# takah29/3d-reconstruction-from-multi-view-exp

Measured on AMD Instinct MI355X. Metric: BA iterations/sec + residual-Jacobian GObs/s, 1M pts x 100 cams fp64, higher is better.
Workload: dtype f64

## Files before the change

3d-reconstruction-from-multi-view-exp_amd/csrc/host_check.cpp:

```cpp
#include <algorithm>
#include <cmath>
#include <cstdio>
#include <cstring>
#include <iterator>
#include <limits>
#include <string>
#include <vector>

#include "mvba_host.h"
#include "mvba_engine_host.h"
#include "mvba_ransac_host.h"
#include "mvba_tracks_host.h"
#include "mvba_match_host.h"

namespace mvba {
thread_local std::string g_err;
}
using namespace mvba;

static int failures = 0;
#define CHECK(x) do { if (!(x)) { std::printf("host_check: line %d: %s\n", __LINE__, #x); ++failures; } } while (0)

int main() {
  {
// ... 796 lines not shown
    auto cost_threads = [](int m) { return std::min(512, table_block_threads(sizeof(double) * (size_t)CAM_LDS * m)); };
    CHECK(k5_bytes(182) == 40768 && k5_bytes(183) == 40992 && k5_bytes(365) == 81760 && k5_bytes(366) == 81984);
    CHECK(table_block_threads(k5_bytes(182)) == 256 && table_block_threads(k5_bytes(183)) == 512);
    CHECK(table_block_threads(k5_bytes(365)) == 512 && table_block_threads(k5_bytes(366)) == 1024);
    CHECK(table_block_threads(40 * 1024) == 256 && table_block_threads(80 * 1024) == 512 && table_block_threads(0) == 256);
    CHECK(cost_threads(284) == 256 && cost_threads(285) == 512 && cost_threads(646) == 512);
    CHECK(k5_lanes(40.0) == 2 && k5_lanes(std::nextafter(40.0, 41.0)) == 4 && k5_lanes(100.0) == 4 && k5_lanes(std::nextafter(100.0, 101.0)) == 8 && k5_lanes(1.0) == 2);
    CHECK(cov_lanes(12.0) == 8 && cov_lanes(std::nextafter(12.0, 13.0)) == 16 && cov_lanes(24.0) == 16 && cov_lanes(std::nextafter(24.0, 25.0)) == 32);
    CHECK(cov_lanes(48.0) == 32 && cov_lanes(std::nextafter(48.0, 49.0)) == 64 && cov_lanes(0.0) == 8);
    auto in = [](auto &dom, int v) { return std::find(std::begin(dom), std::end(dom), v) != std::end(dom); };
    for (double d : {1.0, 40.0, 41.0, 100.0, 101.0, 1e6}) CHECK(in(K5_LANES, k5_lanes(d)));
    for (size_t by : {(size_t)0, (size_t)40961, (size_t)81921, (size_t)160 * 1024}) CHECK(in(TABLE_BLOCK_THREADS, table_block_threads(by)));
    for (double pr : {0.0, 13.0, 25.0, 49.0, 1e6}) CHECK(in(COV_LANES, cov_lanes(pr)));
    CHECK(std::size(K5_LANES) == 3 && std::size(TABLE_BLOCK_THREADS) == 3 && std::size(COV_LANES) == 4);
  }
  if (failures) return 1;
  std::printf("host_check ok\n");
  return 0;
}
```

3d-reconstruction-from-multi-view-exp_amd/csrc/mvba_create.h:

```cpp

__global__ __launch_bounds__(256) void k_xy_from_planes(const double2 *__restrict__ planes, long long N, int m, double2 *__restrict__ xy) {
  const long long a = (long long)blockIdx.x * 256 + threadIdx.x;
  const int k = blockIdx.y;
  if (a < N) xy[a * m + k] = planes[(long long)k * N + a];
}

#define CR(x) do { int rc_ = (x); if (rc_) return rc_; } while (0)

struct CreateTimer {
  bool on;
  std::chrono::steady_clock::time_point t_last = std::chrono::steady_clock::now();
  void lap(const char *what) {
    if (!on) return;
    const auto now = std::chrono::steady_clock::now();
    fprintf(stderr, "mvba_create: %-28s %8.1f ms\n", what, std::chrono::duration<double, std::milli>(now - t_last).count());
    t_last = now;
  }
};

int validate_problem(const mvba_problem *p, std::vector<int> &obs_pt) {
  if (p->n_points < 0 || p->n_images < 2 || p->n_obs < 0 || !p->pt_ptr || (p->n_obs && (!p->cam_idx || !p->xy)))
    return fail(MVBA_ERR_BADARG, "bad problem sizes or null arrays (need n_images >= 2)");
  if (p->gauge_axis != 0 && p->gauge_axis != 1) return fail(MVBA_ERR_BADARG, "gauge_axis must be 0 or 1");
  if (p->xy_layout != 0 && p->xy_layout != 1) return fail(MVBA_ERR_BADARG, "xy_layout must be 0 (observation order) or 1 (image planes)");
// ... 121 lines not shown
    L.n_diag_lists += L.S[pair_id(m, k, k)];
    for (int l = k + 1; l < m; ++l) L.n_off_lists += L.S[pair_id(m, k, l)];
  }
  L.vp_off.assign(L.VP + 1, 0);
  for (long long q = 0; q < P; ++q)
    for (int sI = 0; sI < L.S[q]; ++sI) L.vp_off[L.vp_ptr[q] + sI + 1] = (L.cnt[q] - sI + L.S[q] - 1) / L.S[q];
  for (int v = 0; v < L.VP; ++v) L.vp_off[v + 1] += L.vp_off[v];
  return MVBA_OK;
}

struct PointRanges {
  int nR = 1;
  std::vector<long long> lo;
};

PointRanges make_ranges(const IndexInput &in, const PairLists &L, bool slots, int xcd_waves, int W) {
  PointRanges R;
  const long long N = in.N;
  if (slots) {
    const long long j = std::max<long long>(1, std::min<long long>(xcd_waves / std::max(1LL, L.slot_waves(W)), L.target / (8 * 64)));
    R.nR = (int)(8 * std::min<long long>(j, 8));
    R.lo.assign(R.nR + 1, 0);
    std::vector<long long> pre(N + 1, 0);
    for (long long a = 0; a < N; ++a) {
      const long long d = in.p->pt_ptr[a + 1] - in.p->pt_ptr[a];
      pre[a + 1] = pre[a] + d * (d + 1) / 2;
    }
    for (int r = 0; r <= R.nR; ++r)
      R.lo[r] = std::lower_bound(pre.begin(), pre.end(), (long long)((__int128)pre[N] * r / R.nR)) - pre.begin();
    R.lo[0] = 0; R.lo[R.nR] = N;
  } else {
    const long long nR_big = (L.target + L.unit_items / 2) / L.unit_items, nR_fill = std::min<long long>((4096 + L.VP - 1) / L.VP, L.target / 128);
    R.nR = (int)std::max<long long>(1, std::min<long long>(64, std::max(nR_big, nR_fill)));
    R.lo.assign(R.nR + 1, 0);
    for (int r = 0; r <= R.nR; ++r) R.lo[r] = (long long)((__int128)N * r / R.nR);
  }
  return R;
}

constexpr long long LANES_SKEW = 12288;
constexpr long long LANES_MIN_WAVES = 78;

struct SchurPlan {
  int mode = SCHUR_SLOTS;
  int W = PSTEP;
  std::vector<int> dense_obs;
  PairLists L;
  PointRanges R;
};

template <typename CountPairs>
int decide_schur_form(const IndexInput &in, const CreateKnobs &knobs, int loss, int device, CountPairs count_pairs, SchurPlan &plan,
                      CreateTimer &timer) {
  const mvba_problem *p = in.p;
  const long long N = in.N, nobs = in.nobs;
  const int m = in.m;
  {
    bool few = m >= 1 && 9 * m <= 16 * DENSE_MAX_TILES && N > 0, full = few && nobs == N * (long long)m;
    for (long long a = 0; a < N && full; ++a) {
      if (p->pt_ptr[a + 1] - p->pt_ptr[a] != m) { full = false; break; }
      const int *ci = p->cam_idx + p->pt_ptr[a];
      for (int k = 0; k < m; ++k)
        if (ci[k] != k) { full = false; break; }
    }
    const bool forced = knobs.schur_dense;
    bool masked = few && !full && (forced || (!knobs.schur_set && (double)nobs >= 0.6 * (double)N * m)) && (long long)N * m < (1LL << 31);
    if (masked) {
      plan.dense_obs.assign((size_t)N * m, -1);
// ... 9 lines not shown
    if ((full && (!knobs.schur_set || forced)) || masked) {
      plan.mode = SCHUR_DENSE;
      return MVBA_OK;
    }
  }
  plan.L.cnt.assign(in.P, 0);
  CR(count_pairs(plan.L.cnt));
  timer.lap("pair counts");
  CR(size_pair_lists(in, plan.L));
  const PairLists &L = plan.L;
  int n_cu_dev = 256;
  hipDeviceGetAttribute(&n_cu_dev, hipDeviceAttributeMultiprocessorCount, device);
  auto xcd_waves = [&](int W) { return std::max(1, n_cu_dev / 8) * (W == LANES_W ? 160 * 1024 / LANES_LDS : 160 * 1024 / SLOT_LDS); };
  const bool slots_forced = knobs.schur_slots || knobs.schur_lanes;
  const bool may_slots = !knobs.schur_pairs && loss == LOSS_SQUARED && (N + 1) * 128LL < (1LL << 32) && !knobs.force_big && (L.T >= 4000000 || slots_forced);
  auto slot_plan = [&](int W, PointRanges &R) {
    if (!may_slots || L.slot_waves(W) > xcd_waves(W)) return false;
    R = make_ranges(in, L, true, xcd_waves(W), W);
    if (W == PSTEP && !slots_forced && R.nR * L.slot_waves(W) < 512) return false;
    long long widest = 0;
    for (int r = 0; r < R.nR; ++r) widest = std::max<long long>(widest, p->pt_ptr[R.lo[r + 1]] - p->pt_ptr[R.lo[r]]);
    return (widest + 1) * 128LL < (1LL << 32);
  };
  PointRanges R21, R64;
  const bool fits21 = slot_plan(PSTEP, R21);
  const bool lanes = knobs.schur_lanes ? slot_plan(LANES_W, R64)
                                       : (fits21 && !knobs.schur_slots && L.slot_waves(LANES_W) >= LANES_MIN_WAVES && slot_plan(LANES_W, R64));
  if (lanes) {
    plan.mode = SCHUR_SLOTS; plan.W = LANES_W; plan.R = std::move(R64);
  } else if (fits21) {
    plan.mode = SCHUR_SLOTS; plan.W = PSTEP; plan.R = std::move(R21);
  } else {
    plan.mode = SCHUR_PAIRS;
    plan.R = make_ranges(in, L, false, 0, PSTEP);
  }
  return MVBA_OK;
}
// ... 559 lines not shown
  MVBA_HIP(hipGetDevice(&h->device));
  MVBA_HIP(hipStreamCreateWithFlags(&h->stream, hipStreamNonBlocking));
  CR(h->mem.alloc(&h->d_pt_ptr, N + 1));
  CR(h->mem.alloc(&h->d_cam, nobs));
  MVBA_HIP(hipMemcpy(h->d_pt_ptr, p->pt_ptr, sizeof(long long) * (N + 1), hipMemcpyHostToDevice));
  if (nobs) MVBA_HIP(hipMemcpy(h->d_cam, p->cam_idx, sizeof(int) * nobs, hipMemcpyHostToDevice));
  timer.lap("device, topology upload");
  h->k1_threads = k1_block_threads(m, h->gcam);

  const bool dev_build = N > 0 && nobs > 0 && !knobs.index_host;
  const IndexInput in{p, N, nobs, (long long)m * (m + 1) / 2, m,
                      (int)std::max(1u, std::min({std::thread::hardware_concurrency(), 16u, (unsigned)m})), h->stream, h->d_pt_ptr, h->d_cam};
  DeviceIndexBuild dv;
  SchurPlan plan;
  SchurIndex ix;
  CR(decide_schur_form(in, knobs, h->loss, h->device, [&](std::vector<long long> &cnt) {
    return dev_build ? count_pairs_device(in, knobs, dv, cnt) : count_pairs_host(in, cnt);
  }, plan, timer));
  h->schur_mode = plan.mode;
  h->use_pairs = plan.mode != SCHUR_DENSE;
  h->rec_compact = plan.mode == SCHUR_SLOTS && plan.W == LANES_W && h->loss == LOSS_SQUARED && !h->gcam && !knobs.rec_full;
  if (h->use_pairs) CR(dev_build ? build_index_device(in, plan, dv, h->mem, ix, timer) : build_index_host(in, plan, h->mem, ix, timer));
  timer.lap("queues / wave descriptors");

  CR(alloc_engine_buffers(h, tiles));
  timer.lap("allocations");
  CR(upload_engine(h, p, obs_pt, tiles, plan, ix));
  timer.lap("uploads");
  CR(set_kernel_attributes(h, knobs));
  timer.lap("attributes");
  return MVBA_OK;
}

int create_engine(const mvba_problem *p, int loss, double loss_b, mvba_handle **out) {
  if (!p || !out) return fail(MVBA_ERR_BADARG, "null argument");
  const CreateKnobs knobs = read_create_knobs();
// ... 27 lines not shown
```

3d-reconstruction-from-multi-view-exp_amd/csrc/mvba_debug.h:

```cpp
#include <functional>

extern "C" {

namespace {
constexpr int SNAP_SLAB = 8;
size_t snap_stride(const mvba_handle *h) { return (3 * (size_t)h->N + (size_t)CAM_IN * h->m + 1) & ~(size_t)1; }
double *snap_entry(const mvba_handle *h, long long i) { return h->snap_slabs[(size_t)(i / SNAP_SLAB)] + snap_stride(h) * (size_t)(i % SNAP_SLAB); }
}

int mvba_snapshot(mvba_handle *h) {
  if (!h) return fail(MVBA_ERR_BADARG, "null handle");
  if (!h->have_params) return fail(MVBA_ERR_STATE, "no parameters set");
  MVBA_HIP(hipSetDevice(h->device));
  if ((size_t)(h->n_snap / SNAP_SLAB) >= h->snap_slabs.size()) {
    double *p = nullptr;
    int rc = h->mem.alloc(&p, snap_stride(h) * SNAP_SLAB);
    if (rc) return rc;
    h->snap_slabs.push_back(p);
  }
  double *dst = snap_entry(h, h->n_snap);
  MVBA_HIP(hipMemcpyAsync(dst, h->d_X[h->cur], sizeof(double) * 3 * h->N, hipMemcpyDeviceToDevice, h->stream));
  MVBA_HIP(hipMemcpyAsync(dst + 3 * h->N, h->d_cam15[h->cur], sizeof(double) * CAM_IN * h->m, hipMemcpyDeviceToDevice, h->stream));
  h->n_snap++;
  return MVBA_OK;
// ... 36 lines not shown
int mvba_get_stats(mvba_handle *h, mvba_stats *out) {
  if (!h || !out) return fail(MVBA_ERR_BADARG, "null argument");
  MVBA_HIP(hipSetDevice(h->device));
  int rc = sync_and_drain(h);
  if (rc) return rc;
  *out = h->stats;
  return MVBA_OK;
}

int mvba_get_info(mvba_handle *h, int64_t *out8) {
  if (!h || !out8) return fail(MVBA_ERR_BADARG, "null argument");
  out8[0] = h->n_items;
  out8[1] = h->n_items_offdiag;
  out8[2] = h->n_units;
  out8[3] = h->schur_mode | (h->schur_mode == SCHUR_SLOTS ? h->slot_w << 8 : 0) | (h->rec_compact ? 1 << 16 : 0) |
            (h->schur_mode == SCHUR_DENSE ? (int64_t)h->dense_blocks << 32 : 0);
  out8[4] = h->rccl_version;
  out8[5] = NCCL_VERSION_CODE;
  out8[6] = h->nranks;
  out8[7] = h->schur_mode == SCHUR_SLOTS ? h->n_slot_items : 0;
  return MVBA_OK;
}

int mvba_reset_stats(mvba_handle *h) {
  if (!h) return fail(MVBA_ERR_BADARG, "null handle");
  MVBA_HIP(hipSetDevice(h->device));
  int rc = sync_and_drain(h);
  if (rc) return rc;
  h->stats = mvba_stats{};
  return MVBA_OK;
// ... 54 lines not shown
}

int debug_fill_A(mvba_handle *h, double *out) {
  std::vector<double> pk(h->n_A());
  MVBA_HIP(hipMemcpy(pk.data(), h->d_Ab, sizeof(double) * pk.size(), hipMemcpyDeviceToHost));
  expand_packed_A(pk.data(), h->m, out);
  return MVBA_OK;
}

int debug_fill_index(mvba_handle *h, int which, long long cnt, double *out) {
  if (h->schur_mode == SCHUR_SLOTS && which != MVBA_BUF_INDEX_SEG) {
    const int W = h->slot_w, row = slot_idx_ints(W);
    const long long n_steps = cnt / W;
    std::vector<int> tmp((size_t)n_steps * row);
    if (cnt) MVBA_HIP(hipMemcpy(tmp.data(), h->d_it_x, sizeof(int) * tmp.size(), hipMemcpyDeviceToHost));
    const int off = which == MVBA_BUF_INDEX_K ? 0 : (which == MVBA_BUF_INDEX_L ? W : 2 * W);
    for (long long st = 0; st < n_steps; ++st)
      for (int sl = 0; sl < W; ++sl) out[st * W + sl] = (double)tmp[(size_t)st * row + off + sl];
    return MVBA_OK;
  }
  const int *src = which == MVBA_BUF_INDEX_K ? h->d_it_k : (which == MVBA_BUF_INDEX_L ? h->d_it_l : (which == MVBA_BUF_INDEX_A ? h->d_it_a : h->d_seg_end));
  std::vector<int> tmp((size_t)cnt);
  if (cnt) MVBA_HIP(hipMemcpy(tmp.data(), src, sizeof(int) * tmp.size(), hipMemcpyDeviceToHost));
  for (long long i = 0; i < cnt; ++i) out[i] = (double)tmp[i];
  return MVBA_OK;
}

DebugBuf debug_buffer(mvba_handle *h, int which) {
  const long long N = h->N, nobs = h->nobs, n9 = (long long)h->n9();
  switch (which) {
// ... 36 lines not shown
```

3d-reconstruction-from-multi-view-exp_amd/csrc/mvba_engine.h:

```cpp
enum { SCHUR_PAIRS = 1, SCHUR_SLOTS = 2, SCHUR_DENSE = 3 };
struct mvba_handle {
  int device = 0;
  hipStream_t stream = nullptr;
  DevBufs mem;
  long long N = 0, nobs = 0;
  int m = 0, gauge_axis = 0, D = 0, ld = 0;
  double f0 = 1.0;
  long long *d_pt_ptr = nullptr;
  int *d_cam = nullptr, *d_obs_pt = nullptr;
  double2 *d_xy = nullptr;
  int *d_tiles = nullptr;
  int *d_tile_slot = nullptr;
  int4 *d_splits = nullptr;
  double *d_PLsplit = nullptr;
  int n_splits = 0;
  int n_tiles = 0;
  bool any_split = false;
  int k1_threads = 512;
  bool gcam = false;
  double *d_cam18 = nullptr, *d_dxi10 = nullptr;
  bool use_pairs = true;
  int schur_mode = 2;
  bool index_on_device = false;
  bool force_big = false;
  long long n_items = 0, n_items_offdiag = 0, n_slot_items = 0;
  int n_units = 0, q_max = 0;
  int *d_it_k = nullptr, *d_it_l = nullptr, *d_it_a = nullptr, *d_unit_ptr = nullptr, *d_q_ptr = nullptr, *d_q_units = nullptr;
  int4 *d_units = nullptr;
  double *d_partial = nullptr;
  int n_waves = 0, slot_nR = 8, slot_nseg = 0;
  int slot_w = PSTEP;
  long long *d_range_o0 = nullptr;
  int *d_seg_end = nullptr, *d_prog = nullptr;
  int4 *d_wdesc = nullptr;
  int *d_it_x = nullptr;
  int *d_wunits = nullptr;
  double *d_dense_part = nullptr;
  int *d_dense_obs = nullptr;
  int dense_blocks = 0, dense_tiles = 0;
  double *d_X[2] = {nullptr, nullptr}, *d_cam15[2] = {nullptr, nullptr};
  int cur = 0;
  bool have_params = false, linearized = false, have_trial = false;
  double *d_sim = nullptr;
  double2 *d_rec = nullptr;
  bool rec_compact = false;
  double2 *d_res = nullptr, *d_rec_full = nullptr;
// ... 261 lines not shown
  const size_t lds = cam_lds_bytes(h->m, h->gcam, false);
  cam_tables(h, cam15, nullptr);
  launch_loss(h, cost_kernel(h->gcam, h->loss), dim3(h->cost_grid), dim3(std::min(512, table_block_threads(lds))), lds, h->nobs, h->m, cam15, X,
              h->d_obs_pt, h->d_cam, h->d_xy, h->f0, h->d_partials, h->d_cam18);
  double *mail = cost_mail(h);
  const unsigned long long seq = h->cost_seq;
  hipLaunchKernelGGL(k_sum_partials, dim3(1), dim3(1024), 0, h->stream, h->d_partials, h->cost_grid, h->d_cost, h->d_flag, mail, seq);
  MVBA_HIP(hipGetLastError());
  return MVBA_OK;
}

struct CreateKnobs {
  bool schur_set = false;
  bool schur_slots = false, schur_lanes = false, schur_pairs = false, schur_dense = false;
  bool index_host = false, index_global = false;
  bool force_big = false;
  bool rec_full = false;
  bool chol_launches = false;
  int trail64_min = 200;
  unsigned barrier_polls = 1u << 22;
  bool check_solve = false;
  double check_solve_tol = 1e-8;
  bool timing = false;
};

CreateKnobs read_create_knobs() {
  CreateKnobs k;
  auto is = [](const char *ev, const char *v) { return ev && !strcmp(ev, v); };
  const char *schur = getenv("MVBA_SCHUR");
  k.schur_set = schur != nullptr;
  k.schur_slots = is(schur, "slots");
  k.schur_lanes = is(schur, "lanes");
  k.schur_pairs = is(schur, "pairs");
  k.schur_dense = is(schur, "dense");
  const char *index = getenv("MVBA_INDEX");
  k.index_host = is(index, "host");
  k.index_global = is(index, "global");
  k.force_big = getenv("MVBA_FORCE_BIG") != nullptr;
  k.rec_full = is(getenv("MVBA_REC"), "full");
  k.chol_launches = is(getenv("MVBA_CHOL"), "launches");
  if (const char *ev = getenv("MVBA_TRAIL64_MIN")) k.trail64_min = std::max(0, atoi(ev));
  if (const char *ev = getenv("MVBA_CHOL_BARRIER_POLLS")) k.barrier_polls = (unsigned)std::max(0LL, atoll(ev));
  if (const char *ev = getenv("MVBA_CHECK_SOLVE")) {
    const double v = atof(ev);
    k.check_solve = v != 0.0;
    if (v > 0.0 && v < 1.0) k.check_solve_tol = v;
  }
  k.timing = getenv("MVBA_CREATE_TIMING") != nullptr;
  return k;
}

}
// ... 1 lines not shown
```

3d-reconstruction-from-multi-view-exp_amd/csrc/mvba_engine_host.h:

```cpp
#pragma once
#include <algorithm>
#include <cmath>
#include <cstddef>
#include <string>
#include <vector>

#include "mvba_common.h"

namespace mvba {

inline bool is_gauge_slot(long long g, int axis) { return (g >= 3 && g <= 8) || g == 12 + axis; }

struct ParameterMap {
  bool is_default = false;
  std::vector<int> ptr, mem;
  std::vector<int2> pairs;
  int U = 0, nblk = 1;
};

inline int build_parameter_map(const int32_t *col, int m, int axis, int n_free, int D, ParameterMap &out) {
  const int n9 = 9 * m;
  if (n_free < 0 || n_free > D)
    return fail(MVBA_ERR_BADARG, "mvba_set_parameter_map: n_free = " + std::to_string(n_free) + " must be in 0 .. 9 n_images - 7 = " + std::to_string(D));
  std::vector<int> cnt(n_free + 1, 0), first(n_free, -1);
// ... 109 lines not shown
    double *c = cam + (size_t)k * CAM_IN;
    c[0] = f[k]; c[1] = u[2 * k]; c[2] = u[2 * k + 1];
    for (int i = 0; i < 3; ++i) c[3 + i] = t[3 * k + i];
    for (int i = 0; i < 9; ++i) c[6 + i] = R[9 * k + i];
  }
}
inline void unpack_cam15(const double *cam , int m, double *f, double *u, double *t, double *R) {
  for (int k = 0; k < m; ++k) {
    const double *c = cam + (size_t)k * CAM_IN;
    f[k] = c[0]; u[2 * k] = c[1]; u[2 * k + 1] = c[2];
    for (int i = 0; i < 3; ++i) t[3 * k + i] = c[3 + i];
    for (int i = 0; i < 9; ++i) R[9 * k + i] = c[6 + i];
  }
}

constexpr int K5_LANES[] = {2, 4, 8};
inline int k5_lanes(double mean_degree) { return mean_degree <= 40.0 ? 2 : (mean_degree <= 100.0 ? 4 : 8); }
constexpr int TABLE_BLOCK_THREADS[] = {256, 512, 1024};
inline int table_block_threads(size_t lds_bytes) { return lds_bytes > 80 * 1024 ? 1024 : (lds_bytes > 40 * 1024 ? 512 : 256); }
constexpr int COV_LANES[] = {8, 16, 32, 64};
inline int cov_lanes(double mean_pairs) { return mean_pairs > 48.0 ? 64 : (mean_pairs > 24.0 ? 32 : (mean_pairs > 12.0 ? 16 : 8)); }

}
```

3d-reconstruction-from-multi-view-exp_amd/csrc/mvba_index.h:

```cpp

constexpr int IDX_WAVES = 4;

__device__ __forceinline__ int idx_pair_id(int k, int l, int m) { return k * m - k * (k - 1) / 2 + (l - k); }

template <bool GLOBAL>
__global__ __launch_bounds__(64 * IDX_WAVES) void k_idx_count(long long N, int m, int P, const long long *__restrict__ pt_ptr,
                                                              const int *__restrict__ cam_idx, int chunk,
                                                              int *__restrict__ hist, const int *__restrict__ order) {
  extern __shared__ int s_hist_all[];
  const int lane = threadIdx.x & 63, wv = threadIdx.x >> 6;
  const long long w = (long long)blockIdx.x * IDX_WAVES + wv;
  int *s_hist = GLOBAL ? hist + (size_t)w * P : s_hist_all + (size_t)wv * P;
  if (!GLOBAL) {
    for (int q = lane; q < P; q += 64) s_hist[q] = 0;
    wave_sync();
  }
  const long long a0 = w * chunk, a1 = min(N, a0 + chunk);
  for (long long ai = a0; ai < a1; ++ai) {
    const long long a = order ? order[ai] : ai;
    const long long o0 = pt_ptr[a];
    const int d = (int)(pt_ptr[a + 1] - o0);
    for (int i = 0; i < d; ++i) {
      const int k = cam_idx[o0 + i];
      for (int j = i + lane; j < d; j += 64) {
// ... 121 lines not shown
  }
  if (FILL) {
    if (lane == 0)
      while (sg < nSeg) seg_end[b * nSeg + sg++] = steps;
  } else if (lane == 0) {
    w_steps[b] = steps;
  }
}

__global__ void k_idx_interleave(long long n_steps, int W, int row, const int *__restrict__ st_k, const int *__restrict__ st_l,
                                 const int *__restrict__ st_a, int *__restrict__ out) {
  const long long t = (long long)blockIdx.x * blockDim.x + threadIdx.x;
  if (t >= n_steps * row) return;
  const long long st = t / row;
  const int e = (int)(t - st * row), which = e / W, sl = e - which * W;
  const int *src = which == 0 ? st_k : (which == 1 ? st_l : st_a);
  out[t] = which < 3 ? src[st * W + sl] : 0;
}
```

3d-reconstruction-from-multi-view-exp_amd/csrc/mvba_lanes.h:

```cpp
#pragma once

constexpr int LANES_W = 64;
constexpr int LANES_IDX = 3 * LANES_W;
constexpr int LANES_BUF = SchurStage<LANES_W, false, true>::SIZE;
constexpr int LANES_LDS = 3 * LANES_BUF + 2 * LANES_IDX * 4;
static_assert(LANES_BUF == 17408 && LANES_LDS == 53760, "the launch's LDS bytes");
static_assert(SchurStage<LANES_W, true, true>::SIZE <= LANES_BUF, "a diagonal step fits the buffer");
static_assert(3 * ((LANES_LDS + 511) / 512 * 512) <= 160 * 1024, "three waves per CU");
constexpr int LANES_BUF_C = SchurStage<LANES_W, false, true, true>::SIZE;
constexpr int LANES_LDS_C = 3 * LANES_BUF_C + 2 * LANES_IDX * 4;
static_assert(LANES_BUF_C == 13312 && LANES_LDS_C == 41472, "the compact launch's LDS bytes");
static_assert(SchurStage<LANES_W, true, true, true>::SIZE == 12288, "a compact diagonal step fits the buffer");
static_assert(3 * ((LANES_LDS_C + 511) / 512 * 512) <= 160 * 1024 && 4 * ((LANES_LDS_C + 511) / 512 * 512) > 160 * 1024, "three waves per CU");

struct LanesCompact {
  const double2 *res = nullptr;
  const int4 *units = nullptr;
  const double *cam15 = nullptr;
};
template <int SH>
__device__ __forceinline__ void lds_gather16_rows(int row, unsigned slot16, const void *base, unsigned lds) {
  unsigned o;
  asm volatile("s_mov_b32 m0, %4\n\tv_lshl_add_u32 %0, %1, %5, %2\n\tglobal_load_lds_dwordx4 %0, %3" : "=&v"(o) : "v"(row), "v"(slot16), "s"(base), "s"(lds), "i"(SH) : "memory");
}
template <int G>
__device__ __forceinline__ void lanes_wait() {
  static_assert(G == 12 || G == 13 || G == 17, "the loops of k_schur_lanes and k_schur_lanes_compact");
  if (G == 12) asm volatile("s_waitcnt vmcnt(12)" ::: "memory");
// ... 9 lines not shown
  using S = SchurStage<LANES_W, DIAG, true, COMPACT>;
  constexpr int NPS = S::NPS, BUFSZ = S::SIZE, NBUF = 3;
  constexpr int RSL = COMPACT ? 4 : 7;
  constexpr int G = DIAG ? RSL + 1 + NPS : RSL + RSL + NPS;
  double acc[9][9];
#pragma unroll
  for (int i = 0; i < 9; ++i)
#pragma unroll
    for (int j = 0; j < 9; ++j) acc[i][j] = 0.0;
  double dg[9], rb[9];
#pragma unroll
  for (int j = 0; j < 9; ++j) dg[j] = rb[j] = 0.0;

  const unsigned lds0 = (unsigned)(unsigned long long)(__attribute__((address_space(3))) char *)wbuf;
  const unsigned ldsx0 = lds0 + NBUF * BUFSZ;
  const int *xring = reinterpret_cast<const int *>(wbuf + NBUF * BUFSZ);
  const int *xbase = it_x + beg * LANES_IDX;
  const int last_st = nst - 1;
  auto rec_row = [&](int j) { return (64 * j + lane) / RSL; };
  auto rec_s16 = [&](int j) { return COMPACT ? (unsigned)((lane & 3) ^ ((lane >> 4) & 3)) << 4 : (unsigned)((64 * j + lane) % 7) << 4; };
  auto pb_row = [&](int j) { return (64 * j + lane) / NPS; };
  auto pb_s16 = [&](int j) { return (unsigned)(COMPACT ? ((64 * j + lane) % NPS + 6) & 7 : (64 * j + lane) % NPS) << 4; };
  const unsigned lane16 = (unsigned)min(lane, 47) << 4;
  auto index_row = [&](int st, unsigned ring_off) {
    const int *src = xbase + (size_t)min(st, last_st) * LANES_IDX;
    const unsigned dst = ldsx0 + ring_off;
    if (lane < 48) lds_index_row(lane16, src, dst);
  };
  constexpr unsigned RING_B = LANES_IDX * 4;
  auto issue_step = [&](unsigned ring_off, unsigned ring_next, unsigned buf_off, int st_idx) {
    index_row(st_idx, ring_next);
    const int *x = reinterpret_cast<const int *>(reinterpret_cast<const char *>(xring) + ring_off);
    const unsigned buf = lds0 + buf_off;
    int kx[RSL], ax[NPS], lx[RSL];
#pragma unroll
    for (int j = 0; j < RSL; ++j) kx[j] = x[rec_row(j)];
#pragma unroll
    for (int j = 0; j < NPS; ++j) ax[j] = x[2 * LANES_W + pb_row(j)];
#pragma unroll
    for (int j = 0; j < RSL; ++j) lx[j] = DIAG ? (j == 0 ? x[lane] : 0) : x[LANES_W + rec_row(j)];
#pragma unroll
    for (int j = 0; j < RSL; ++j) asm volatile("" : "+v"(kx[j]), "+v"(lx[j]));
#pragma unroll
    for (int j = 0; j < NPS; ++j) asm volatile("" : "+v"(ax[j]));
    if constexpr (COMPACT) {
#pragma unroll
      for (int j = 0; j < RSL; ++j) {
        lds_gather16_rows<6>(kx[j], rec_s16(j), rec, buf + 1024 * j);
        if (!DIAG) lds_gather16_rows<6>(lx[j], rec_s16(j), rec, buf + S::L + 1024 * j);
      }
      if (DIAG) lds_gather16_rows<4>(lx[0], 0u, cx.res, buf + S::L);
    } else if (!DIAG) {
#pragma unroll
      for (int j = 0; j < 7; ++j) {
        lds_gather16(kx[j], rec_s16(j), rec, buf + 1024 * j);
        lds_gather16(lx[j], rec_s16(j), rec, buf + S::L + 1024 * j);
      }
    } else {
#pragma unroll
// ... 118 lines not shown
```

3d-reconstruction-from-multi-view-exp_amd/csrc/mvba_schur.h:

```cpp


constexpr int PSTEP = 21;
constexpr int PROW = 7 * 16;
constexpr int UNIT_STRIDE = 104;
constexpr int SLOT_IDX = 64;
constexpr int SLOT_IDX_RING = 3;

template <int W, bool DIAG, bool PACKED, bool COMPACT = false>
struct SchurStage {
  static_assert(!COMPACT || PACKED, "the compact rows are the slot forms'");
  static constexpr int ROW = COMPACT ? 4 * 16 : PROW;
  static constexpr int NPS = (DIAG ? 5 : 3) + (COMPACT ? 2 : 0);
  static constexpr int L = W * ROW;
  static constexpr int P = L + ((PACKED && DIAG) ? W * 16 : W * ROW);
  static constexpr int SIZE = P + W * 16 * (PACKED ? NPS : 5);
  static constexpr int SQW = DIAG ? L + W * 16 : P + W * 16 * NPS;
  static constexpr int SQW_END = SQW + (DIAG ? 1 : 2) * W * 8;
};
constexpr int PWAVE_LDS = SchurStage<PSTEP, false, false>::SIZE;
constexpr int SLOT_BUF = SchurStage<PSTEP, false, true>::SIZE;
constexpr int PAIRS_LDS = 2 * PWAVE_LDS;
constexpr int SLOT_LDS = 3 * SLOT_BUF + SLOT_IDX_RING * SLOT_IDX * 4;
static_assert(PWAVE_LDS == 6384 && SLOT_BUF == 5712 && SLOT_LDS == 17904, "the launches' LDS bytes");
static_assert(SchurStage<PSTEP, true, false>::SIZE == PWAVE_LDS && SchurStage<PSTEP, true, true>::SIZE <= SLOT_BUF, "a diagonal step fits the buffer");
// ... 428 lines not shown
      double *__restrict__ partial, int nR, const int *__restrict__ seg_end, int *__restrict__ prog,                      \
      int nseg, int lag, const long long *__restrict__ range_o0
__global__ __launch_bounds__(64, 3) void k_schur_slots(MVBA_SLOTS_ARGS) {
  schur_slots_wave(wdesc, wunits, it_k, it_l, it_a, rec, PB, c, f0, partial, nR, seg_end, prog, nseg, lag, range_o0);
}

#include "mvba_lanes.h"
constexpr int slot_idx_ints(int W) { return W == LANES_W ? LANES_IDX : SLOT_IDX; }

__global__ __launch_bounds__(64, 1) void k_schur_lanes(const int4 *__restrict__ wdesc, const int *__restrict__ wunits,
                                                       const int *__restrict__ it_x, const double2 *__restrict__ rec,
                                                       const double *__restrict__ PB, double c, double f0,
                                                       double *__restrict__ partial, int nR,
                                                       const long long *__restrict__ range_o0) {
  extern __shared__ char smem_pairs[];
  const int bid = blockIdx.x;
  const int MVBA_CONST_AS *dp = as_const(reinterpret_cast<const int *>(wdesc)) + 4 * (size_t)bid;
  const int d_x = dp[0], d_y = dp[1], nsteps = dp[2], flags = dp[3];
  if (nsteps <= 0) return;
  const long long beg = ((long long)d_y << 32) | (unsigned)d_x;
  const int *su = wunits + (size_t)bid * LANES_W;
  const double2 *rec_r = rec + (size_t)as_const(range_o0)[bid % nR] * REC;
  if (flags & 1) schur_lanes_run<true>(smem_pairs, (int)threadIdx.x, beg, nsteps, it_x, rec_r, PB, c, 1.0 / f0, partial, su);
  else schur_lanes_run<false>(smem_pairs, (int)threadIdx.x, beg, nsteps, it_x, rec_r, PB, c, 1.0 / f0, partial, su);
}
__global__ __launch_bounds__(64, 1) void k_schur_lanes_compact(const int4 *__restrict__ wdesc, const int *__restrict__ wunits,
                                                               const int *__restrict__ it_x, const double2 *__restrict__ rec,
                                                               const double *__restrict__ PB, double c, double f0,
                                                               double *__restrict__ partial, int nR,
                                                               const long long *__restrict__ range_o0, const double2 *__restrict__ res,
                                                               const int4 *__restrict__ units, const double *__restrict__ cam15) {
  extern __shared__ char smem_pairs[];
  const int bid = blockIdx.x;
  const int MVBA_CONST_AS *dp = as_const(reinterpret_cast<const int *>(wdesc)) + 4 * (size_t)bid;
  const int d_x = dp[0], d_y = dp[1], nsteps = dp[2], flags = dp[3];
  if (nsteps <= 0) return;
  const long long beg = ((long long)d_y << 32) | (unsigned)d_x;
  const int *su = wunits + (size_t)bid * LANES_W;
  const long long o0 = as_const(range_o0)[bid % nR];
  const LanesCompact cx{res + o0, units, cam15};
  if (flags & 1) schur_lanes_run<true, true>(smem_pairs, (int)threadIdx.x, beg, nsteps, it_x, rec + (size_t)o0 * REC_C, PB, c, 1.0 / f0, partial, su, cx);
  else schur_lanes_run<false, true>(smem_pairs, (int)threadIdx.x, beg, nsteps, it_x, rec + (size_t)o0 * REC_C, PB, c, 1.0 / f0, partial, su, cx);
}

__global__ __launch_bounds__(128) void k_schur_reduce(int m, const int *__restrict__ unit_ptr,
                                                      const double *__restrict__ partial, double *__restrict__ Afull,
                                                      double *__restrict__ bfull) {
  const long long p = blockIdx.x;
// ... 32 lines not shown
```

3d-reconstruction-from-multi-view-exp_amd/lib/_mvba.py:

```python
from __future__ import annotations

import ctypes as C
import os
import threading

import numpy as np

_HERE = os.path.dirname(os.path.abspath(__file__))
LIB_PATH = os.environ.get("MVBA_LIBRARY", os.path.join(os.path.dirname(_HERE), "libmvba.so"))

MVBA_OK, MVBA_ERR_BADARG, MVBA_ERR_SINGULAR, MVBA_ERR_HIP, MVBA_ERR_RCCL, MVBA_ERR_STATE = range(6)

KERNEL_IDS = ("resid_jac", "point_blocks", "point_inv", "schur", "allreduce", "solve", "backsub_cost", "cost")
BUF = {"residual": 0, "JX": 1, "JC": 2, "E": 3, "dP": 4, "A_full": 5, "b_full": 6, "dxi": 7, "dX": 8,
       "trial_X": 9, "trial_cam": 10, "index_k": 11, "index_l": 12, "index_a": 13, "index_seg": 14, "weight": 15}
LOSSES = {"squared": 0, "huber": 1, "cauchy": 2}


def check_loss(loss, loss_scale):
    if not isinstance(loss, str) or loss not in LOSSES:
        raise ValueError(f"loss must be one of {sorted(LOSSES)}, got {loss!r}")
    if loss == "squared":
        return 0, 0.0
    if loss_scale is None:
# ... 367 lines not shown
        raise_for(self.lib.mvba_get_stats(self._h, C.byref(s)), self.lib)
        out = {k: {"ms": s.ms[i], "launches": s.launches[i]} for i, k in enumerate(KERNEL_IDS)}
        out["counts"] = {"linearize": s.n_linearize, "try_step": s.n_try_step, "commit": s.n_commit,
                         "lu_fallback": s.n_lu_fallback, "barrier_fallback": s.n_barrier_fallback}
        return out

    def _info(self):
        out = (C.c_int64 * 8)()
        raise_for(self.lib.mvba_get_info(self._h, out), self.lib)
        return list(out)

    def schur_info(self):
        i = self._info()
        return {"items": i[0], "offdiag_items": i[1], "units": i[2], "kernel": ("strip", "pairs", "slots", "dense")[i[3] & 0xff],
                "slot_rows": i[7], "step_width": (i[3] >> 8) & 0xff,
                "record": "compact" if (i[3] >> 16) & 1 else "full",
                "workgroups": i[3] >> 32}

    def rccl_version(self):
        i = self._info()
        return {"loaded": i[4], "compiled_against": i[5], "ranks": i[6]}

    def comm_init(self, id128: bytes, rank: int, n_ranks: int):
        buf = C.create_string_buffer(bytes(id128), 128)
        raise_for(self.lib.mvba_comm_init(self._h, buf, int(rank), int(n_ranks)), self.lib)

    def comm_init_host(self, rank: int, n_ranks: int, allreduce):
        HOSTFN = C.CFUNCTYPE(C.c_int, C.c_void_p, _dp, C.c_int64)

        def _cb(_user, buf, n):
# ... 544 lines not shown
```

Before: 453.8.

## Pack lane Schur indices into two words and size ranges by occupancy

The (k, l, a) index triple for each 64-wide lane step is packed into two 32-bit words instead of three. This shrinks the per-block LDS index ring so the compact lanes kernel fits four waves per CU instead of three. The number of point ranges is now derived from the measured occupancy (blocks per CU times CU count) rather than a fixed multiple of eight. Blocks are remapped to range waves so that each range stays on its home XCD. The cost is extra bit unpacking per step, a range limit on N and degree for the packed format, and a lower LANES_MIN_WAVES threshold that may change which Schur kernel is selected.

After: 486.9 (median of 6 runs). +7.3%, better.

```diff
diff --git a/3d-reconstruction-from-multi-view-exp_amd/csrc/host_check.cpp b/3d-reconstruction-from-multi-view-exp_amd/csrc/host_check.cpp
--- a/3d-reconstruction-from-multi-view-exp_amd/csrc/host_check.cpp
+++ b/3d-reconstruction-from-multi-view-exp_amd/csrc/host_check.cpp
@@ -834,6 +834,72 @@
     for (double pr : {0.0, 13.0, 25.0, 49.0, 1e6}) CHECK(in(COV_LANES, cov_lanes(pr)));
     CHECK(std::size(K5_LANES) == 3 && std::size(TABLE_BLOCK_THREADS) == 3 && std::size(COV_LANES) == 4);
   }
+  {
+    const int ROW = (int)LANE_IDX_MAX_ROW, OFF = (int)LANE_IDX_MAX_OFF;
+    CHECK(LANE_IDX_ROW_BITS == 25 && LANE_IDX_OFF_BITS == 14 && ROW == (1 << 25) - 1 && OFF == 16383);
+    auto round_trip = [](int k, int l, int a) {
+      int k2 = -1, l2 = -1, a2 = -1;
+      const LaneIdx p = lane_idx_pack(k, l, a);
+      lane_idx_unpack(p, k2, l2, a2);
+      return k2 == k && l2 == l && a2 == a && lane_idx_k(p.w0) == k && lane_idx_l(p.w0, p.w1) == l && lane_idx_a(p.w1) == a;
+    };
+    const int ks[] = {0, 1, 127, 128, (1 << 24) + 5, ROW - OFF, ROW - 1, ROW}, as[] = {0, 1, 77, 1 << 24, ROW - 1, ROW};
+    const int ds[] = {0, 1, 63, 64, 79, 127, 128, 129, 255, 256, 8191, 8192, OFF - 1, OFF};
+    for (int k : ks)
+      for (int d : ds)
+        for (int a : as)
+          if ((long long)k + d <= ROW) CHECK(round_trip(k, k + d, a));
+    CHECK(round_trip(ROW - OFF, ROW, ROW));
+    {
+      const int N = 1234567;
+      const LaneIdx pad = lane_idx_pack(0, 0, N), dg = lane_idx_pack(4711, 4711, 42);
+      CHECK(pad.w0 == 0u && pad.w1 == (unsigned)N && round_trip(0, 0, N) && round_trip(0, 0, ROW));
+      CHECK(dg.w0 == 4711u && dg.w1 == 42u && lane_idx_l(dg.w0, dg.w1) == lane_idx_k(dg.w0));
+    }
+    CHECK(lane_idx_pack(0, 127, 0).w0 == 127u << 25 && lane_idx_pack(0, 127, 0).w1 == 0u);
+    CHECK(lane_idx_pack(0, 128, 0).w0 == 0u && lane_idx_pack(0, 128, 0).w1 == 1u << 25);
+    CHECK(lane_idx_pack(ROW - OFF, ROW, ROW).w1 == 0xffffffffu);
+    static_assert(lane_idx_l(lane_idx_pack(5, 300, 9).w0, lane_idx_pack(5, 300, 9).w1) == 300, "constexpr on the host and in the kernels");
+    const long long NMAX = (1LL << 32) / 128 - 2;
+    CHECK((NMAX + 1) * 128 < (1LL << 32) && (NMAX + 2) * 128 >= (1LL << 32));
+    CHECK(lane_idx_fits(NMAX, NMAX, 16384) && !lane_idx_fits(NMAX, NMAX, 16385) && lane_idx_fits(0, 0, 0) && lane_idx_fits(10, 20, 1));
+    CHECK(!lane_idx_fits(ROW + 1, 10, 2) && !lane_idx_fits(10, ROW + 2, 2) && lane_idx_fits(ROW, ROW + 1, 2));
+  }
+  {
+    const long long T = 10000;
+    CHECK(lane_ranges(1024, 95, T, 0) == 10 && lane_ranges(768, 95, T, 0) == 8);
+    CHECK(lane_ranges(1024, 78, T, 0) == 13 && lane_ranges(1024, 63, T, 0) == 16 && lane_ranges(1024, 96, T, 0) == 10);
+    CHECK(lane_ranges(1024, 1024, T, 0) == 1 && lane_ranges(1024, 1025, T, 0) == 1 && lane_ranges(1024, 513, T, 0) == 1 && lane_ranges(1024, 512, T, 0) == 2);
+    CHECK(lane_ranges(1000, 96, T, 0) == 10 && lane_ranges(959, 96, T, 0) == 9);
+    CHECK(lane_ranges(1024, 1, T, 0) == 64 && lane_ranges(1024, 9, 1LL << 40, 0) == 64 && lane_ranges(1024, 9, 1024, 0) == 16 && lane_ranges(1024, 9, 1023, 0) == 8);
+    CHECK(lane_ranges(1024, 9, 0, 0) == 8 && lane_ranges(1024, 200, 0, 0) == 5 && lane_ranges(0, 9, T, 0) == 1 && lane_ranges(1024, 0, T, 0) == 64);
+    CHECK(lane_ranges(1024, 95, T, 1) == 1 && lane_ranges(1024, 95, T, 3) == 3 && lane_ranges(1024, 95, T, 11) == 11 && lane_ranges(768, 95, 0, 64) == 64);
+    CHECK(lane_ranges(1024, 95, T, 65) == LANE_MAX_RANGES && lane_ranges(1024, 95, T, 1 << 30) == LANE_MAX_RANGES);
+  }
+  {
+    for (int nR : {1, 3, 7, 8, 9, 10, 11, 15, 16, 17, 23, 64})
+      for (int rw : {1, 2, 9, 95, 96}) {
+        const int T = nR * rw, q = nR / 8;
+        std::vector<int> seen(T, 0), surplus(8, 0);
+        bool home_ok = true, same = true, order = true;
+        std::vector<int> last_w(nR, -1);
+        for (int B = 0; B < T; ++B) {
+          const int b = lane_wave_of_block(B, nR, rw);
+          if (b < 0 || b >= T) { home_ok = false; continue; }
+          ++seen[b];
+          const int r = b % nR, w = b / nR;
+          if (r < 8 * q) home_ok = home_ok && B % 8 == r % 8;
+          else ++surplus[B % 8];
+          same = same && b == B;
+          order = order && w > last_w[r];
+          last_w[r] = w;
+        }
+        CHECK(std::all_of(seen.begin(), seen.end(), [](int c) { return c == 1; }));
+        CHECK(home_ok && order);
+        CHECK(*std::max_element(surplus.begin(), surplus.end()) - *std::min_element(surplus.begin(), surplus.end()) <= 1);
+        CHECK(same || (nR % 8 != 0 && nR > 8));
+      }
+  }
   if (failures) return 1;
   std::printf("host_check ok\n");
   return 0;
diff --git a/3d-reconstruction-from-multi-view-exp_amd/csrc/mvba_create.h b/3d-reconstruction-from-multi-view-exp_amd/csrc/mvba_create.h
--- a/3d-reconstruction-from-multi-view-exp_amd/csrc/mvba_create.h
+++ b/3d-reconstruction-from-multi-view-exp_amd/csrc/mvba_create.h
@@ -159,12 +159,12 @@
   std::vector<long long> lo;
 };
 
-PointRanges make_ranges(const IndexInput &in, const PairLists &L, bool slots, int xcd_waves, int W) {
+PointRanges make_ranges(const IndexInput &in, const PairLists &L, bool slots, int xcd_waves, int W, int lane_nR = 0) {
   PointRanges R;
   const long long N = in.N;
   if (slots) {
     const long long j = std::max<long long>(1, std::min<long long>(xcd_waves / std::max(1LL, L.slot_waves(W)), L.target / (8 * 64)));
-    R.nR = (int)(8 * std::min<long long>(j, 8));
+    R.nR = W == LANES_W ? std::max(1, lane_nR) : (int)(8 * std::min<long long>(j, 8));
     R.lo.assign(R.nR + 1, 0);
     std::vector<long long> pre(N + 1, 0);
     for (long long a = 0; a < N; ++a) {
@@ -184,7 +184,7 @@
 }
 
 constexpr long long LANES_SKEW = 12288;
-constexpr long long LANES_MIN_WAVES = 78;
+constexpr long long LANES_MIN_WAVES = 38;
 
 struct SchurPlan {
   int mode = SCHUR_SLOTS;
@@ -192,11 +192,12 @@
   std::vector<int> dense_obs;
   PairLists L;
   PointRanges R;
+  int lane_places = 0;
 };
 
 template <typename CountPairs>
-int decide_schur_form(const IndexInput &in, const CreateKnobs &knobs, int loss, int device, CountPairs count_pairs, SchurPlan &plan,
-                      CreateTimer &timer) {
+int decide_schur_form(const IndexInput &in, const CreateKnobs &knobs, int loss, bool compact_rec, int device, CountPairs count_pairs,
+                      SchurPlan &plan, CreateTimer &timer) {
   const mvba_problem *p = in.p;
   const long long N = in.N, nobs = in.nobs;
   const int m = in.m;
@@ -236,13 +237,23 @@
   auto xcd_waves = [&](int W) { return std::max(1, n_cu_dev / 8) * (W == LANES_W ? 160 * 1024 / LANES_LDS : 160 * 1024 / SLOT_LDS); };
   const bool slots_forced = knobs.schur_slots || knobs.schur_lanes;
   const bool may_slots = !knobs.schur_pairs && loss == LOSS_SQUARED && (N + 1) * 128LL < (1LL << 32) && !knobs.force_big && (L.T >= 4000000 || slots_forced);
+  int lane_places = 0;
+  if (may_slots)
+    MVBA_HIP(hipOccupancyMaxActiveBlocksPerMultiprocessor(&lane_places, compact_rec ? (const void *)k_schur_lanes_compact : (const void *)k_schur_lanes, 64,
+                                                          compact_rec ? LANES_LDS_C : LANES_LDS));
+  lane_places = std::max(1, lane_places);
+  plan.lane_places = lane_places;
+  long long max_degree = 0;
+  for (long long a = 0; a < N; ++a) max_degree = std::max<long long>(max_degree, p->pt_ptr[a + 1] - p->pt_ptr[a]);
   auto slot_plan = [&](int W, PointRanges &R) {
     if (!may_slots || L.slot_waves(W) > xcd_waves(W)) return false;
-    R = make_ranges(in, L, true, xcd_waves(W), W);
+    R = make_ranges(in, L, true, xcd_waves(W), W,
+                    lane_ranges((long long)n_cu_dev * lane_places, L.slot_waves(LANES_W), L.target, knobs.slot_ranges));
     if (W == PSTEP && !slots_forced && R.nR * L.slot_waves(W) < 512) return false;
     long long widest = 0;
     for (int r = 0; r < R.nR; ++r) widest = std::max<long long>(widest, p->pt_ptr[R.lo[r + 1]] - p->pt_ptr[R.lo[r]]);
-    return (widest + 1) * 128LL < (1LL << 32);
+    if ((widest + 1) * 128LL >= (1LL << 32)) return false;
+    return W != LANES_W || lane_idx_fits(N, widest, max_degree);
   };
   PointRanges R21, R64;
   const bool fits21 = slot_plan(PSTEP, R21);
@@ -832,12 +843,14 @@
   DeviceIndexBuild dv;
   SchurPlan plan;
   SchurIndex ix;
-  CR(decide_schur_form(in, knobs, h->loss, h->device, [&](std::vector<long long> &cnt) {
+  const bool compact_rec = h->loss == LOSS_SQUARED && !h->gcam && !knobs.rec_full;
+  CR(decide_schur_form(in, knobs, h->loss, compact_rec, h->device, [&](std::vector<long long> &cnt) {
     return dev_build ? count_pairs_device(in, knobs, dv, cnt) : count_pairs_host(in, cnt);
   }, plan, timer));
   h->schur_mode = plan.mode;
   h->use_pairs = plan.mode != SCHUR_DENSE;
-  h->rec_compact = plan.mode == SCHUR_SLOTS && plan.W == LANES_W && h->loss == LOSS_SQUARED && !h->gcam && !knobs.rec_full;
+  h->rec_compact = plan.mode == SCHUR_SLOTS && plan.W == LANES_W && compact_rec;
+  h->lane_places = plan.mode == SCHUR_SLOTS && plan.W == LANES_W ? plan.lane_places : 0;
   if (h->use_pairs) CR(dev_build ? build_index_device(in, plan, dv, h->mem, ix, timer) : build_index_host(in, plan, h->mem, ix, timer));
   timer.lap("queues / wave descriptors");
 
diff --git a/3d-reconstruction-from-multi-view-exp_amd/csrc/mvba_debug.h b/3d-reconstruction-from-multi-view-exp_amd/csrc/mvba_debug.h
--- a/3d-reconstruction-from-multi-view-exp_amd/csrc/mvba_debug.h
+++ b/3d-reconstruction-from-multi-view-exp_amd/csrc/mvba_debug.h
@@ -74,6 +74,7 @@
   out8[1] = h->n_items_offdiag;
   out8[2] = h->n_units;
   out8[3] = h->schur_mode | (h->schur_mode == SCHUR_SLOTS ? h->slot_w << 8 : 0) | (h->rec_compact ? 1 << 16 : 0) |
+            (h->schur_mode == SCHUR_SLOTS ? (int64_t)(h->slot_nR & 0xff) << 20 | (int64_t)(h->lane_places & 0xf) << 28 : 0) |
             (h->schur_mode == SCHUR_DENSE ? (int64_t)h->dense_blocks << 32 : 0);
   out8[4] = h->rccl_version;
   out8[5] = NCCL_VERSION_CODE;
@@ -158,6 +159,15 @@
     const long long n_steps = cnt / W;
     std::vector<int> tmp((size_t)n_steps * row);
     if (cnt) MVBA_HIP(hipMemcpy(tmp.data(), h->d_it_x, sizeof(int) * tmp.size(), hipMemcpyDeviceToHost));
+    if (W == LANES_W) {
+      for (long long st = 0; st < n_steps; ++st)
+        for (int sl = 0; sl < W; ++sl) {
+          int k, l, a;
+          lane_idx_unpack({(unsigned)tmp[(size_t)st * row + sl], (unsigned)tmp[(size_t)st * row + W + sl]}, k, l, a);
+          out[st * W + sl] = (double)(which == MVBA_BUF_INDEX_K ? k : (which == MVBA_BUF_INDEX_L ? l : a));
+        }
+      return MVBA_OK;
+    }
     const int off = which == MVBA_BUF_INDEX_K ? 0 : (which == MVBA_BUF_INDEX_L ? W : 2 * W);
     for (long long st = 0; st < n_steps; ++st)
       for (int sl = 0; sl < W; ++sl) out[st * W + sl] = (double)tmp[(size_t)st * row + off + sl];
diff --git a/3d-reconstruction-from-multi-view-exp_amd/csrc/mvba_engine.h b/3d-reconstruction-from-multi-view-exp_amd/csrc/mvba_engine.h
--- a/3d-reconstruction-from-multi-view-exp_amd/csrc/mvba_engine.h
+++ b/3d-reconstruction-from-multi-view-exp_amd/csrc/mvba_engine.h
@@ -30,6 +30,7 @@
   double *d_partial = nullptr;
   int n_waves = 0, slot_nR = 8, slot_nseg = 0;
   int slot_w = PSTEP;
+  int lane_places = 0;
   long long *d_range_o0 = nullptr;
   int *d_seg_end = nullptr, *d_prog = nullptr;
   int4 *d_wdesc = nullptr;
@@ -321,6 +322,7 @@
   bool schur_set = false;
   bool schur_slots = false, schur_lanes = false, schur_pairs = false, schur_dense = false;
   bool index_host = false, index_global = false;
+  int slot_ranges = 0;
   bool force_big = false;
   bool rec_full = false;
   bool chol_launches = false;
@@ -343,6 +345,7 @@
   const char *index = getenv("MVBA_INDEX");
   k.index_host = is(index, "host");
   k.index_global = is(index, "global");
+  if (const char *ev = getenv("MVBA_SLOT_RANGES")) k.slot_ranges = std::max(0, atoi(ev));
   k.force_big = getenv("MVBA_FORCE_BIG") != nullptr;
   k.rec_full = is(getenv("MVBA_REC"), "full");
   k.chol_launches = is(getenv("MVBA_CHOL"), "launches");
diff --git a/3d-reconstruction-from-multi-view-exp_amd/csrc/mvba_engine_host.h b/3d-reconstruction-from-multi-view-exp_amd/csrc/mvba_engine_host.h
--- a/3d-reconstruction-from-multi-view-exp_amd/csrc/mvba_engine_host.h
+++ b/3d-reconstruction-from-multi-view-exp_amd/csrc/mvba_engine_host.h
@@ -147,6 +147,41 @@
   }
 }
 
+constexpr int LANE_IDX_ROW_BITS = 25, LANE_IDX_OFF_BITS = 2 * (32 - LANE_IDX_ROW_BITS);
+constexpr unsigned LANE_IDX_ROW_MASK = (1u << LANE_IDX_ROW_BITS) - 1, LANE_IDX_OFF_LOW = (1u << (32 - LANE_IDX_ROW_BITS)) - 1;
+constexpr long long LANE_IDX_MAX_ROW = LANE_IDX_ROW_MASK, LANE_IDX_MAX_OFF = (1LL << LANE_IDX_OFF_BITS) - 1;
+struct LaneIdx { unsigned w0, w1; };
+__host__ __device__ constexpr LaneIdx lane_idx_pack(int k, int l, int a) {
+  const unsigned d = (unsigned)(l - k);
+  return {(unsigned)k | (d & LANE_IDX_OFF_LOW) << LANE_IDX_ROW_BITS, (unsigned)a | (d >> (32 - LANE_IDX_ROW_BITS)) << LANE_IDX_ROW_BITS};
+}
+__host__ __device__ constexpr int lane_idx_k(unsigned w0) { return (int)(w0 & LANE_IDX_ROW_MASK); }
+__host__ __device__ constexpr int lane_idx_a(unsigned w1) { return (int)(w1 & LANE_IDX_ROW_MASK); }
+__host__ __device__ constexpr int lane_idx_l(unsigned w0, unsigned w1) {
+  return (int)((w0 & LANE_IDX_ROW_MASK) + (w0 >> LANE_IDX_ROW_BITS) + ((w1 >> LANE_IDX_ROW_BITS) << (32 - LANE_IDX_ROW_BITS)));
+}
+__host__ __device__ constexpr void lane_idx_unpack(LaneIdx p, int &k, int &l, int &a) {
+  k = lane_idx_k(p.w0); l = lane_idx_l(p.w0, p.w1); a = lane_idx_a(p.w1);
+}
+constexpr bool lane_idx_fits(long long N, long long widest, long long max_degree) {
+  return N <= LANE_IDX_MAX_ROW && widest - 1 <= LANE_IDX_MAX_ROW && max_degree - 1 <= LANE_IDX_MAX_OFF;
+}
+static_assert((1LL << 32) / 128 - 2 <= LANE_IDX_MAX_ROW, "the largest N (and range) with (N + 1) * 128 < 2^32 fits the row fields");
+
+constexpr int LANE_MAX_RANGES = 64;
+inline int lane_ranges(long long places, long long range_waves, long long target, int forced) {
+  if (forced > 0) return std::min(forced, LANE_MAX_RANGES);
+  const long long cap = 8 * std::max<long long>(1, std::min<long long>(LANE_MAX_RANGES / 8, target / (8 * 64)));
+  return (int)std::max<long long>(1, std::min(places / std::max<long long>(1, range_waves), cap));
+}
+
+__host__ __device__ constexpr int lane_wave_of_block(int B, int nR, int range_waves) {
+  const int q = nR / 8, s = nR - 8 * q, i = B / 8, x = B % 8, home = q * range_waves;
+  if (i < home) return nR * (i / q) + x + 8 * (i % q);
+  const int j = 8 * (i - home) + x;
+  return nR * (j / s) + 8 * q + j % s;
+}
+
 constexpr int K5_LANES[] = {2, 4, 8};
 inline int k5_lanes(double mean_degree) { return mean_degree <= 40.0 ? 2 : (mean_degree <= 100.0 ? 4 : 8); }
 constexpr int TABLE_BLOCK_THREADS[] = {256, 512, 1024};
diff --git a/3d-reconstruction-from-multi-view-exp_amd/csrc/mvba_index.h b/3d-reconstruction-from-multi-view-exp_amd/csrc/mvba_index.h
--- a/3d-reconstruction-from-multi-view-exp_amd/csrc/mvba_index.h
+++ b/3d-reconstruction-from-multi-view-exp_amd/csrc/mvba_index.h
@@ -159,6 +159,12 @@
   if (t >= n_steps * row) return;
   const long long st = t / row;
   const int e = (int)(t - st * row), which = e / W, sl = e - which * W;
+  if (W == LANES_W) {
+    const long long o = st * W + sl;
+    const LaneIdx p = lane_idx_pack(st_k[o], st_l[o], st_a[o]);
+    out[t] = (int)(which == 0 ? p.w0 : p.w1);
+    return;
+  }
   const int *src = which == 0 ? st_k : (which == 1 ? st_l : st_a);
   out[t] = which < 3 ? src[st * W + sl] : 0;
 }
diff --git a/3d-reconstruction-from-multi-view-exp_amd/csrc/mvba_lanes.h b/3d-reconstruction-from-multi-view-exp_amd/csrc/mvba_lanes.h
--- a/3d-reconstruction-from-multi-view-exp_amd/csrc/mvba_lanes.h
+++ b/3d-reconstruction-from-multi-view-exp_amd/csrc/mvba_lanes.h
@@ -1,17 +1,17 @@
 #pragma once
 
 constexpr int LANES_W = 64;
-constexpr int LANES_IDX = 3 * LANES_W;
+constexpr int LANES_IDX = 2 * LANES_W;
 constexpr int LANES_BUF = SchurStage<LANES_W, false, true>::SIZE;
 constexpr int LANES_LDS = 3 * LANES_BUF + 2 * LANES_IDX * 4;
-static_assert(LANES_BUF == 17408 && LANES_LDS == 53760, "the launch's LDS bytes");
+static_assert(LANES_BUF == 17408 && LANES_LDS == 53248, "the launch's LDS bytes");
 static_assert(SchurStage<LANES_W, true, true>::SIZE <= LANES_BUF, "a diagonal step fits the buffer");
-static_assert(3 * ((LANES_LDS + 511) / 512 * 512) <= 160 * 1024, "three waves per CU");
+static_assert(3 * ((LANES_LDS + 511) / 512 * 512) <= 160 * 1024 && 4 * ((LANES_LDS + 511) / 512 * 512) > 160 * 1024, "three waves per CU");
 constexpr int LANES_BUF_C = SchurStage<LANES_W, false, true, true>::SIZE;
 constexpr int LANES_LDS_C = 3 * LANES_BUF_C + 2 * LANES_IDX * 4;
-static_assert(LANES_BUF_C == 13312 && LANES_LDS_C == 41472, "the compact launch's LDS bytes");
+static_assert(LANES_BUF_C == 13312 && LANES_LDS_C == 40960, "the compact launch's LDS bytes");
 static_assert(SchurStage<LANES_W, true, true, true>::SIZE == 12288, "a compact diagonal step fits the buffer");
-static_assert(3 * ((LANES_LDS_C + 511) / 512 * 512) <= 160 * 1024 && 4 * ((LANES_LDS_C + 511) / 512 * 512) > 160 * 1024, "three waves per CU");
+static_assert(4 * ((LANES_LDS_C + 511) / 512 * 512) <= 160 * 1024 && 5 * ((LANES_LDS_C + 511) / 512 * 512) > 160 * 1024, "four waves per CU, one per SIMD");
 
 struct LanesCompact {
   const double2 *res = nullptr;
@@ -51,35 +51,43 @@
 
   const unsigned lds0 = (unsigned)(unsigned long long)(__attribute__((address_space(3))) char *)wbuf;
   const unsigned ldsx0 = lds0 + NBUF * BUFSZ;
-  const int *xring = reinterpret_cast<const int *>(wbuf + NBUF * BUFSZ);
+  const unsigned *xring = reinterpret_cast<const unsigned *>(wbuf + NBUF * BUFSZ);
   const int *xbase = it_x + beg * LANES_IDX;
   const int last_st = nst - 1;
   auto rec_row = [&](int j) { return (64 * j + lane) / RSL; };
   auto rec_s16 = [&](int j) { return COMPACT ? (unsigned)((lane & 3) ^ ((lane >> 4) & 3)) << 4 : (unsigned)((64 * j + lane) % 7) << 4; };
   auto pb_row = [&](int j) { return (64 * j + lane) / NPS; };
   auto pb_s16 = [&](int j) { return (unsigned)(COMPACT ? ((64 * j + lane) % NPS + 6) & 7 : (64 * j + lane) % NPS) << 4; };
-  const unsigned lane16 = (unsigned)min(lane, 47) << 4;
+  const unsigned lane16 = (unsigned)min(lane, 31) << 4;
   auto index_row = [&](int st, unsigned ring_off) {
     const int *src = xbase + (size_t)min(st, last_st) * LANES_IDX;
     const unsigned dst = ldsx0 + ring_off;
-    if (lane < 48) lds_index_row(lane16, src, dst);
+    if (lane < 32) lds_index_row(lane16, src, dst);
   };
   constexpr unsigned RING_B = LANES_IDX * 4;
   auto issue_step = [&](unsigned ring_off, unsigned ring_next, unsigned buf_off, int st_idx) {
     index_row(st_idx, ring_next);
-    const int *x = reinterpret_cast<const int *>(reinterpret_cast<const char *>(xring) + ring_off);
+    const unsigned *x = reinterpret_cast<const unsigned *>(reinterpret_cast<const char *>(xring) + ring_off);
     const unsigned buf = lds0 + buf_off;
+    unsigned k0[RSL], a1[NPS], l1[RSL];
+#pragma unroll
+    for (int j = 0; j < RSL; ++j) k0[j] = x[rec_row(j)];
+#pragma unroll
+    for (int j = 0; j < NPS; ++j) a1[j] = x[LANES_W + pb_row(j)];
+#pragma unroll
+    for (int j = 0; j < RSL; ++j) l1[j] = DIAG ? (j == 0 ? x[lane] : 0u) : x[LANES_W + rec_row(j)];
+#pragma unroll
+    for (int j = 0; j < RSL; ++j) asm volatile("" : "+v"(k0[j]), "+v"(l1[j]));
+#pragma unroll
+    for (int j = 0; j < NPS; ++j) asm volatile("" : "+v"(a1[j]));
     int kx[RSL], ax[NPS], lx[RSL];
 #pragma unroll
-    for (int j = 0; j < RSL; ++j) kx[j] = x[rec_row(j)];
-#pragma unroll
-    for (int j = 0; j < NPS; ++j) ax[j] = x[2 * LANES_W + pb_row(j)];
-#pragma unroll
-    for (int j = 0; j < RSL; ++j) lx[j] = DIAG ? (j == 0 ? x[lane] : 0) : x[LANES_W + rec_row(j)];
-#pragma unroll
-    for (int j = 0; j < RSL; ++j) asm volatile("" : "+v"(kx[j]), "+v"(lx[j]));
-#pragma unroll
-    for (int j = 0; j < NPS; ++j) asm volatile("" : "+v"(ax[j]));
+    for (int j = 0; j < RSL; ++j) {
+      kx[j] = lane_idx_k(k0[j]);
+      lx[j] = DIAG ? (j == 0 ? lane_idx_k(l1[0]) : 0) : lane_idx_l(k0[j], l1[j]);
+    }
+#pragma unroll
+    for (int j = 0; j < NPS; ++j) ax[j] = lane_idx_a(a1[j]);
     if constexpr (COMPACT) {
 #pragma unroll
       for (int j = 0; j < RSL; ++j) {
diff --git a/3d-reconstruction-from-multi-view-exp_amd/csrc/mvba_schur.h b/3d-reconstruction-from-multi-view-exp_amd/csrc/mvba_schur.h
--- a/3d-reconstruction-from-multi-view-exp_amd/csrc/mvba_schur.h
+++ b/3d-reconstruction-from-multi-view-exp_amd/csrc/mvba_schur.h
@@ -466,7 +466,7 @@
                                                        double *__restrict__ partial, int nR,
                                                        const long long *__restrict__ range_o0) {
   extern __shared__ char smem_pairs[];
-  const int bid = blockIdx.x;
+  const int bid = lane_wave_of_block((int)blockIdx.x, nR, (int)gridDim.x / nR);
   const int MVBA_CONST_AS *dp = as_const(reinterpret_cast<const int *>(wdesc)) + 4 * (size_t)bid;
   const int d_x = dp[0], d_y = dp[1], nsteps = dp[2], flags = dp[3];
   if (nsteps <= 0) return;
@@ -483,7 +483,7 @@
                                                                const long long *__restrict__ range_o0, const double2 *__restrict__ res,
                                                                const int4 *__restrict__ units, const double *__restrict__ cam15) {
   extern __shared__ char smem_pairs[];
-  const int bid = blockIdx.x;
+  const int bid = lane_wave_of_block((int)blockIdx.x, nR, (int)gridDim.x / nR);
   const int MVBA_CONST_AS *dp = as_const(reinterpret_cast<const int *>(wdesc)) + 4 * (size_t)bid;
   const int d_x = dp[0], d_y = dp[1], nsteps = dp[2], flags = dp[3];
   if (nsteps <= 0) return;
diff --git a/3d-reconstruction-from-multi-view-exp_amd/lib/_mvba.py b/3d-reconstruction-from-multi-view-exp_amd/lib/_mvba.py
--- a/3d-reconstruction-from-multi-view-exp_amd/lib/_mvba.py
+++ b/3d-reconstruction-from-multi-view-exp_amd/lib/_mvba.py
@@ -405,6 +405,7 @@
         i = self._info()
         return {"items": i[0], "offdiag_items": i[1], "units": i[2], "kernel": ("strip", "pairs", "slots", "dense")[i[3] & 0xff],
                 "slot_rows": i[7], "step_width": (i[3] >> 8) & 0xff,
+                "ranges": (i[3] >> 20) & 0xff, "places_per_cu": (i[3] >> 28) & 0xf,
                 "record": "compact" if (i[3] >> 16) & 1 else "full",
                 "workgroups": i[3] >> 32}
 
```
